# JuanDuGit/DH3D

Measured on AMD Instinct MI355X. Metric: point-clouds/sec, higher is better.
Workload: dtype f32; 1 GPU; local-descriptor forward (basic_config), N=8192 K=8, batch=8; clouds_per_gpu=8, clouds_total=8, points=8192, knn=8, parallelism=clouds sharded over 1 GPU(s), no data-path collective, weights=random-init (no checkpoint blobs exist upstream), steps_in_flight=4

## Files before the change

### dh3d_amd/_lib.py

```python
import ctypes
import os

import torch

_HERE = os.path.dirname(os.path.abspath(__file__))
LIB_PATH = os.environ.get("DH3D_HIP_LIB") or os.path.join(_HERE, "libdh3d_hip.so")

DH3D_OK = 0
ACT_NONE, ACT_RELU, ACT_SIGMOID = 0, 1, 2

_lib = None

c_fp = ctypes.c_void_p
c_int = ctypes.c_int
c_size_t = ctypes.c_size_t
c_float = ctypes.c_float
c_ll = ctypes.c_longlong
c_double = ctypes.c_double
c_u64 = ctypes.c_uint64


class Epilogue(ctypes.Structure):
    _fields_ = [("pre_bias", ctypes.c_void_p), ("scale", ctypes.c_void_p), ("shift", ctypes.c_void_p),
                ("act", ctypes.c_int)]
# ... 76 lines not shown
    "dh3d_netvlad_assign_rows_bwd": [c_fp, c_ll, c_int, c_fp, c_fp, c_fp, c_fp, c_fp, c_fp, c_fp],
    "dh3d_l2norm_rows_bwd": [c_fp, c_fp, c_ll, c_int, c_float, c_fp, c_fp],
    "dh3d_transpose32": [c_fp, c_int, c_int, c_int, c_fp, c_fp],
    "dh3d_colsum_f32": [c_fp, c_ll, c_int, c_int, c_fp, c_fp],
    "dh3d_farthest_point_sample": [c_int, c_int, c_int, c_fp, c_fp, c_fp, c_fp],
    "dh3d_farthest_point_sample_mode": [c_int, c_int, c_int, c_fp, c_fp, c_fp, c_int, c_fp],
    "dh3d_group_point_fwd": [c_int, c_int, c_int, c_int, c_int, c_fp, c_fp, c_fp, c_fp],
    "dh3d_group_point_bwd": [c_int, c_int, c_int, c_int, c_int, c_fp, c_fp, c_fp, c_fp],
    "dh3d_three_nn": [c_int, c_int, c_int, c_fp, c_fp, c_fp, c_fp, c_fp],
    "dh3d_three_interpolate_fwd": [c_int, c_int, c_int, c_int, c_fp, c_fp, c_fp, c_fp, c_fp],
    "dh3d_three_interpolate_bwd": [c_int, c_int, c_int, c_int, c_fp, c_fp, c_fp, c_fp, c_fp],
    "dh3d_spatial_sort": [c_fp, c_int, c_int, c_fp, c_fp, c_fp],
    "dh3d_knn_sorted": [c_fp, c_fp, c_int, c_int, c_int, c_fp, c_fp, c_fp],
    "dh3d_spatial_sort_cells": [c_fp, c_int, c_int, c_fp, c_fp, c_fp, c_fp],
    "dh3d_knn_grid": [c_fp, c_fp, c_fp, c_int, c_int, c_int, c_fp, c_fp, c_fp],
    "dh3d_knn_grid_plan": [c_int, c_int, c_int],
    "dh3d_fps_sorted": [c_fp, c_fp, c_int, c_int, c_int, c_fp, c_fp],
    "dh3d_three_nn_sorted": [c_int, c_int, c_int, c_fp, c_fp, c_fp, c_fp, c_fp, c_fp, c_fp],
    "dh3d_fps_sorted_xyz": [c_fp, c_fp, c_int, c_int, c_int, c_fp, c_fp, c_fp],
    "dh3d_fps_sorted_ordered": [c_fp, c_fp, c_fp, c_int, c_int, c_int, c_fp, c_fp, c_fp, c_fp, c_fp, c_fp],
    "dh3d_fps_sorted_cloud": [c_fp, c_fp, c_fp, c_int, c_int, c_int, c_fp, c_fp, c_fp],
    "dh3d_fps_sorted_fits": [c_int, c_int, c_int, c_int],
    "dh3d_pack_weight": [c_fp, c_int, c_int, c_fp, c_fp],
    "dh3d_pack_flex_weight": [c_fp, c_fp, c_int, c_int, c_fp, c_fp],
    "dh3d_flex_conv_pm_gather_fwd": [c_fp, c_fp, c_int, c_fp, c_fp, c_fp, c_int, c_int, c_int, c_int, c_int,
                                     ctypes.POINTER(Epilogue), c_fp, c_fp],
    "dh3d_flex_conv_pm_fwd": [c_fp, c_fp, c_fp, c_fp, c_int, c_int, c_int, c_int, c_int,
                              ctypes.POINTER(Epilogue), c_fp, c_fp],
    "dh3d_flex_conv_pm_tile_x6_fwd": [c_fp, c_fp, c_fp, c_fp, c_int, c_int, c_int, c_int, c_int, ctypes.POINTER(Epilogue), c_fp,
                                   c_fp, c_int, c_fp, c_fp],
# ... 42 lines not shown
    "dh3d_interp_bn_bwd_sums": [c_fp, c_int, c_int, c_fp, c_fp, c_fp, c_int, c_int, c_int, c_fp, c_fp, c_fp, c_fp, c_fp,
                                c_fp, c_fp, c_fp, c_fp],
    "dh3d_interp_bn_bwd_apply": [c_fp, c_int, c_int, c_fp, c_fp, c_fp, c_int, c_int, c_int, c_fp, c_fp, c_fp, c_fp, c_fp,
                                 c_fp, c_fp, c_fp, c_fp],
    "dh3d_linear_pm_x6_fwd": [c_fp, c_int, c_fp, c_int, c_fp, c_int, c_int, ctypes.POINTER(Epilogue), c_fp, c_fp, c_fp],
    "dh3d_se_res_pm_packed_fwd": [c_fp, c_fp, c_fp, c_fp, c_fp, c_fp, c_int, c_int, c_fp, c_fp],
    "dh3d_se_res_pool_pm_packed_fwd": [c_fp, c_fp, c_int, c_int, c_int, c_fp, c_fp, c_fp, c_fp, c_int, c_fp, c_fp],
    "dh3d_se_res_pool_conv_pm_fwd": [c_fp, c_fp, c_int, c_int, c_int, c_fp, c_fp, c_fp, c_fp, c_int, c_fp, c_fp,
                                     ctypes.POINTER(Epilogue), c_int, c_fp, c_fp],
    "dh3d_flex_pool_pm_fwd": [c_fp, c_fp, c_int, c_int, c_int, c_int, c_fp, c_fp, c_fp],
    "dh3d_flex_avg_pm_fwd": [c_fp, c_fp, c_int, c_int, c_int, c_int, c_float, c_fp, c_fp],
    "dh3d_conv_pointset_pm_fwd": [c_fp, c_fp, c_fp, c_fp, c_int, c_int, c_int, c_int, ctypes.POINTER(Epilogue),
                                  c_fp, c_fp],
    "dh3d_conv_pointset_pool_pm_fwd": [c_fp, c_fp, c_fp, c_fp, c_int, c_int, c_int, c_int, ctypes.POINTER(Epilogue),
                                       c_fp, c_fp, c_fp],
    "dh3d_linear_pm_fwd": [c_fp, c_int, c_fp, c_int, c_fp, c_int, c_int, ctypes.POINTER(Epilogue), c_fp, c_fp,
                           c_fp],
    "dh3d_se_res_pm_fwd": [c_fp, c_fp, c_fp, c_fp, c_fp, c_fp, c_int, c_int, c_fp, c_fp],
    "dh3d_three_interpolate_idw_fwd": [c_int, c_int, c_int, c_int, c_fp, c_fp, c_fp, c_fp, c_fp],
    "dh3d_l2norm_concat_fwd": [c_fp, c_int, c_int, c_float, c_fp, c_int, c_fp, c_fp],
    "dh3d_mlp_head_pm_fwd": [c_fp, c_int, c_int, c_fp, c_int, ctypes.POINTER(Epilogue), c_fp, c_float, c_fp,
                             c_fp],
    "dh3d_pack_weight_x3": [c_fp, c_int, c_int, c_fp, c_fp],
    "dh3d_mlp_head_pm_x6_fwd": [c_fp, c_int, c_int, c_fp, c_int, ctypes.POINTER(Epilogue), c_fp, c_float, c_fp,
                                c_fp],
    "dh3d_netvlad_workspace_bytes": [c_int, c_int, c_int, c_int],
    "dh3d_netvlad_aggregate_fwd": [c_fp, c_fp, c_fp, c_fp, c_fp, c_fp, c_int, c_int, c_int, c_int, c_fp,
                                   c_size_t, c_fp, c_fp],
    "dh3d_netvlad_head_workspace_bytes": [c_int, c_int, c_int],
    "dh3d_netvlad_tail_workspace_bytes": [c_int, c_int, c_int, c_int],
# ... 124 lines not shown
```

### dh3d_amd/backbones.py

```python
import math

import torch
from torch import nn

from . import _lib as L
from . import pm


class TPBatchNorm(nn.Module):

    ema_unbiased = True

    def __init__(self, channels, eps=1e-5):
        super().__init__()
        self.eps = eps
        self.gamma = nn.Parameter(torch.ones(channels))
        self.beta = nn.Parameter(torch.zeros(channels))
        self.register_buffer("mean_EMA", torch.zeros(channels))
        self.register_buffer("variance_EMA", torch.ones(channels))

    def fold(self):
        scale = self.gamma * torch.rsqrt(self.variance_EMA + self.eps)
        shift = self.beta - self.mean_EMA * scale
        return scale.contiguous(), shift.contiguous()
# ... 180 lines not shown
        cp = inner._prep or inner.prepare()
        if (packed is not None and x.dim() == 3 and x.shape[2] == 64 and inner.cin == 64 and inner.cout == 64
                and "wp" in cp and not cp.get("pad")):
            return pm.se_res_pool_conv(x, nbr, *packed, cp["wp"], cp["b"], cp["scale"], cp["shift"], act=act)
        y = self.forward_on_max_pool(x, nbr)
        return y, conv(y, act=act)


class Geometry(object):

    def __init__(self, xyz, knn_num, nbr=None, fps_contract=None):
        self.fps_contract = fps_contract
        self.xyz = xyz
        self.knn_num = knn_num
        self.nbr = nbr
        self.levels = {}
        self.sorted = None
        self.cells = None

    def ordered(self, cells=False):
        if self.sorted is None:
            if cells:
                srt, gbox, self.cells = pm.spatial_sort_cells(self.xyz)
                self.sorted = (srt, gbox)
            else:
                self.sorted = pm.spatial_sort(self.xyz)
        return self.sorted

    def level(self, dilate, knn, finish=True):
        key = (dilate, knn)
# ... 406 lines not shown
```

### dh3d_amd/csrc/flex_pm.hip

```cpp
#include <float.h>

#include "mfma_gemm.h"

namespace {

template <int DIN, int DOUT, int TMSEL = 0>
struct FlexCfg {
  static constexpr int TM = TMSEL ? TMSEL : (DIN <= 64 ? 64 : 32);
  static constexpr int KD = 4 * DIN;
  static constexpr int LD = KD + 4;
  static constexpr int MB = TM / 32;
  static constexpr int NB = DOUT / 32;
  static constexpr int NT = NB * MB / 4;
  static constexpr int LPR = DIN / 4;
  static constexpr int PPR = 256 / LPR;
  static constexpr int ROUNDS = TM / PPR;
  static_assert(NT >= 1 && NB * MB % 4 == 0, "tile must split over 4 waves");
};

template <int DIN, int DOUT, int KT, int TMSEL = 0>
__global__ __launch_bounds__(256) void flex_conv_pm_kernel(
    const float *__restrict__ feat, const float *__restrict__ xyz, const int32_t *__restrict__ nbr,
    const float *__restrict__ wpacked, long long R, int N, int K, EpilogueArgs ep,
    float *__restrict__ out, const int32_t *__restrict__ remap, int Nsrc) {
// ... 421 lines not shown
    hipLaunchKernelGGL(conv_pointset_pm_anyk_kernel, dim3(flat_grid(R * (Dout / 4))), dim3(256), 0,
                       (hipStream_t)stream, xyz, nbr, theta, bias, R, N, K, Dout, dh3d_ep(ep), out);
  }
  return dh3d_launch_status();
}

DH3D_API int dh3d_pointset_sum_pm(const float *xyz, const int32_t *nbr, int B, int N, int K, float *S, void *stream) {
  DH3D_REQUIRE(xyz && nbr && S && B > 0 && N > 0);
  DH3D_SUPPORTED(K == 8);
  const long long R = (long long)B * N;
  hipLaunchKernelGGL(pointset_sum_kernel, dim3(dh3d_cdiv(R, 256)), dim3(256), 0, (hipStream_t)stream, xyz, nbr, R, N,
                     reinterpret_cast<float4 *>(S));
  return dh3d_launch_status();
}

DH3D_API int dh3d_conv_pointset_pool_pm_fwd(const float *xyz, const int32_t *nbr, const float *theta, const float *bias,
                                            int B, int N, int K, int Dout, const dh3d_epilogue *ep, float *scratch,
                                            float *out, void *stream) {
  DH3D_REQUIRE(xyz && nbr && theta && bias && scratch && out && B > 0 && N > 0 && Dout > 0);
  DH3D_SUPPORTED(K == 8 && (Dout == 32 || Dout == 64 || Dout == 128) && (long long)B * N * (Dout / 4) < (1ll << 31));
  const long long R = (long long)B * N;
  hipStream_t s = (hipStream_t)stream;
  float4 *S = reinterpret_cast<float4 *>(scratch);
  hipLaunchKernelGGL(pointset_sum_kernel, dim3(dh3d_cdiv(R, 256)), dim3(256), 0, s, xyz, nbr, R, N, S);
  const dim3 grid(dh3d_cdiv(R * (Dout / 4), 256)), block(256);
  const EpilogueArgs e = dh3d_ep(ep);
  if (Dout == 32)
    hipLaunchKernelGGL(pointset_pool_kernel<8>, grid, block, 0, s, S, nbr, theta, bias, (int)R, N, e, out);
  else if (Dout == 64)
    hipLaunchKernelGGL(pointset_pool_kernel<16>, grid, block, 0, s, S, nbr, theta, bias, (int)R, N, e, out);
  else
    hipLaunchKernelGGL(pointset_pool_kernel<32>, grid, block, 0, s, S, nbr, theta, bias, (int)R, N, e, out);
  return dh3d_launch_status();
}
```

### dh3d_amd/csrc/knn.hip

```cpp
#include <float.h>
#include <limits.h>

#include <type_traits>

#include "common.h"
#include "wave_ops.h"

#pragma clang fp contract(off)

namespace {

typedef float f32x2 __attribute__((ext_vector_type(2)));
typedef unsigned long long u64;

constexpr int kQueriesPerBlock = 256;
constexpr int kChunk = 1024;
constexpr int kQueue = 16;

struct KnnLadder {
  int log2ct;
  int ctmask;
  int cv;
};

// ... 20 lines not shown
__device__ __forceinline__ int cand_slot(int c, int comp) {
  const int g = c >> 2, r = c & 3;
  const int off = (r < 2) ? (2 * comp + r) : (4 + 2 * comp + r);
  return g * 12 + off;
}

__device__ __forceinline__ float knn_bcast(float v, int lane) {
  return __int_as_float(__builtin_amdgcn_readlane(__float_as_int(v), lane));
}

__device__ __forceinline__ int knn_pick_near(unsigned long long m, int gl) {
  const unsigned long long up = m >> gl, dn = m & ((1ull << gl) - 1);
  const int da = up ? __builtin_ctzll(up) : 128;
  const int db = dn ? gl - (63 - __builtin_clzll(dn)) : 128;
  return da <= db ? gl + da : gl - db;
}

template <int KMAX>
struct KnnState {
  u64 keys[KMAX];
  float bound;
};

template <int KMAX, bool KEEP_MIN = false>
__device__ __forceinline__ void knn_insert_key(KnnState<KMAX> &st, const u64 key) {
  if (key < st.keys[KMAX - 1]) {
    if constexpr (KMAX <= 16) {
      bool lt[KMAX];
#pragma unroll
      for (int i = 0; i < KMAX - 1; ++i) lt[i] = key < st.keys[i];
// ... 317 lines not shown
          o_nn[i] = -1;
          o_d[i] = FLT_MAX;
        } else {
          o_nn[i] = (int)(((tb % (unsigned)lad.cv) << lad.log2ct) + tb / (unsigned)lad.cv);
          o_d[i] = __uint_as_float((unsigned)(st.keys[i] >> 32));
        }
      }
    }
  }
}

template <int S>
__host__ __device__ constexpr int knn_split_lds_bytes() {
  return S * (64 * 3 * 4 + kQueue * 64 * 8 + 64 * 4 + 64 * 4 + 64 * 4);
}
template <int KMAX, int S>
__device__ __forceinline__ void knn_split_body(const float4 *__restrict__ sorted, const float *__restrict__ gbox, int N, int K,
                                               const KnnLadder lad, int32_t *__restrict__ nn, float *__restrict__ dist,
                                               const int b, const int g, unsigned char *lds, const int wave0 = 0) {
  static_assert(KMAX * 64 * sizeof(u64) <= kQueue * 64 * sizeof(uint2), "a K-list fits its wave's survivor queue");
  uint2 (*s_q)[kQueue * 64] = reinterpret_cast<uint2 (*)[kQueue * 64]>(lds);
  float (*s_c)[64 * 3] = reinterpret_cast<float (*)[64 * 3]>(lds + S * kQueue * 64 * 8);
  int (*s_id)[64] = reinterpret_cast<int (*)[64]>(lds + S * (kQueue * 64 * 8 + 64 * 3 * 4));
  float (*s_share)[64] = reinterpret_cast<float (*)[64]>(lds + S * (kQueue * 64 * 8 + 64 * 3 * 4 + 64 * 4));
  float (*s_kth)[64] = reinterpret_cast<float (*)[64]>(lds + S * (kQueue * 64 * 8 + 64 * 3 * 4 + 64 * 8));
  constexpr int R = (KMAX + S - 1) / S - 1;
  const int lane = threadIdx.x & 63;
  const int wave = __builtin_amdgcn_readfirstlane((int)(threadIdx.x >> 6) - wave0);
  const int NG = (N + 63) / 64;
  const float4 *sc = sorted + (size_t)b * N;
  const float4 *gb = reinterpret_cast<const float4 *>(gbox) + (size_t)b * NG * 2;
  float *my_c = s_c[wave];
  uint2 *my_q = s_q[wave];
  int *my_id = s_id[wave];
// ... 197 lines not shown
          for (int t = KMAX - 1; t > 0; --t) {
            const u64 a = st.keys[t - 1], c = st.keys[t];
            const bool lt = c < a;
            st.keys[t - 1] = lt ? c : a;
            st.keys[t] = lt ? a : c;
          }
        }
      }
    }
  }

  if (wave == 0 && valid) {
    const int y = __float_as_int(qr.w);
    int32_t *o_nn = nn + ((size_t)b * N + y) * K;
    float *o_d = dist + ((size_t)b * N + y) * K;
#pragma unroll
    for (int i = 0; i < KMAX; ++i) {
      if (i < K) {
        const unsigned tb = (unsigned)st.keys[i];
        if (st.keys[i] == ~0ull) {
          o_nn[i] = -1;
          o_d[i] = FLT_MAX;
        } else {
          o_nn[i] = (int)(((tb % (unsigned)lad.cv) << lad.log2ct) + tb / (unsigned)lad.cv);
          o_d[i] = __uint_as_float((unsigned)(st.keys[i] >> 32));
        }
      }
    }
  }
}


template <int KMAX, int S>
__global__ __launch_bounds__(64 * S) void knn_split_kernel(const float4 *__restrict__ sorted,
                                                         const float *__restrict__ gbox, int N, int K,
                                                         KnnLadder lad, int32_t *__restrict__ nn,
                                                         float *__restrict__ dist, const int *__restrict__ gate) {
  if (gate && !gate[(size_t)blockIdx.y * kCellInts + kCellFlag]) return;
  __shared__ __attribute__((aligned(16))) unsigned char s_lds[knn_split_lds_bytes<S>()];
  const unsigned ng = (unsigned)((N + 63) / 64);
  knn_split_body<KMAX, S>(sorted, gbox, N, K, lad, nn, dist, blockIdx.y, (int)((blockIdx.x + 37u * blockIdx.y) % ng), s_lds);
}
// ... 205 lines not shown
__device__ __forceinline__ unsigned knn_spread4(unsigned v) {
  return (v & 1u) | ((v & 2u) << 2) | ((v & 4u) << 4) | ((v & 8u) << 6);
}
__device__ __forceinline__ void knn_cswap(u64 &a, u64 &b) {
  const bool lt = b < a;
  const u64 lo = lt ? b : a, hi = lt ? a : b;
  a = lo; b = hi;
}
template <int CTRL>
__device__ __forceinline__ u64 knn_dpp_u64(u64 v) {
  const int lo = __builtin_amdgcn_update_dpp(0, (int)(unsigned)v, CTRL, 0xF, 0xF, true);
  const int hi = __builtin_amdgcn_update_dpp(0, (int)(unsigned)(v >> 32), CTRL, 0xF, 0xF, true);
  return ((u64)(unsigned)hi << 32) | (unsigned)lo;
}
template <int CTRL>
__device__ __forceinline__ void knn_merge_step(KnnState<8> &st) {
  u64 c[8];
#pragma unroll
  for (int i = 0; i < 8; ++i) {
    const u64 mine = st.keys[i], theirs = knn_dpp_u64<CTRL>(st.keys[7 - i]);
    c[i] = mine < theirs ? mine : theirs;
  }
  knn_cswap(c[0], c[4]); knn_cswap(c[1], c[5]); knn_cswap(c[2], c[6]); knn_cswap(c[3], c[7]);
  knn_cswap(c[0], c[2]); knn_cswap(c[1], c[3]); knn_cswap(c[4], c[6]); knn_cswap(c[5], c[7]);
  knn_cswap(c[0], c[1]); knn_cswap(c[2], c[3]); knn_cswap(c[4], c[5]); knn_cswap(c[6], c[7]);
#pragma unroll
  for (int i = 0; i < 8; ++i) st.keys[i] = c[i];
}
template <int L>
__device__ __forceinline__ void knn_merge_sublanes(KnnState<8> &st) {
  if (L >= 2) knn_merge_step<0xB1>(st);
  if (L >= 4) knn_merge_step<0x4E>(st);
  if (L >= 8) knn_merge_step<0x141>(st);
  const unsigned hb = (unsigned)(st.keys[7] >> 32);
  if (hb <= 0x7f800000u) {
    const float dk = __uint_as_float(hb);
    st.bound = __fmul_rn(__fmul_rn(dk, dk), 1.000001f);
  }
}

template <int L, int SF>
__global__ __launch_bounds__(256) void knn_grid_kernel(const float4 *__restrict__ sorted, const float *__restrict__ gbox,
                                                      const int *__restrict__ cells, int N, int K, int D, KnnLadder lad,
                                                      int32_t *__restrict__ nn, float *__restrict__ dist) {
  constexpr int QB = 256 / L;
  static_assert(SF == 0 || (L == 4 && SF <= 4), "the merged scan: 64 queries per workgroup, at most four waves");
  constexpr int kGridLds = 3 * 64 * 4 + QB * kGridCap * 2 + QB * 4;
  constexpr int kSplitLds = SF == 2 ? 2 * knn_split_lds_bytes<2>() : SF > 0 ? knn_split_lds_bytes<(SF > 0 ? SF : 1)>() : 0;
  __shared__ __attribute__((aligned(16))) unsigned char s_raw[kGridLds > kSplitLds ? kGridLds : kSplitLds];
  const int b = blockIdx.y, lane = threadIdx.x & 63, sub = lane & (L - 1);
  if (cells[(size_t)b * kCellInts + kCellFlag]) {
    if constexpr (SF > 0) {
      const int ngq = (N + 63) / 64;
      if constexpr (SF == 2) {
        const int half = (int)(threadIdx.x >> 7), pairs = (ngq + 1) / 2;
        if ((int)blockIdx.x >= pairs) return;
        const int g0 = (int)blockIdx.x + half * pairs;
        if (g0 >= ngq) return;
        knn_split_body<8, 2>(sorted, gbox, N, K, lad, nn, dist, b, (int)(((unsigned)g0 + 37u * (unsigned)b) % (unsigned)ngq),
                             s_raw + half * knn_split_lds_bytes<2>(), half * 2);
      } else if (threadIdx.x < 64 * SF) {
        knn_split_body<8, (SF > 0 ? SF : 1)>(sorted, gbox, N, K, lad, nn, dist, b, (int)((blockIdx.x + 37u * (unsigned)b) % (unsigned)ngq), s_raw);
      }
    }
    return;
  }
  const int qi = (int)((blockIdx.x + 37u * (unsigned)b) % gridDim.x) * QB + threadIdx.x / L;
  const bool valid = qi < N;
  const float4 *sc = sorted + (size_t)b * N;
  const int *ct = cells + (size_t)b * kCellInts;
  const float *hd = reinterpret_cast<const float *>(ct) + 4100;
  const float lo[3] = {hd[0], hd[1], hd[2]}, scl[3] = {hd[3], hd[4], hd[5]};
  const float4 qr = sc[valid ? qi : N - 1];
  const float q[3] = {qr.x, qr.y, qr.z};
  const unsigned sched = (unsigned)ct[4107];
  int nb[3] = {0, 0, 0}, drop[3] = {0, 0, 0};
#pragma unroll
// ... 85 lines not shown
  };
  auto drain = [&]() {
    __builtin_amdgcn_fence(__ATOMIC_SEQ_CST, "wavefront");
    __builtin_amdgcn_wave_barrier();
    const int total = min(s_cnt[qs], kGridCap);
#pragma unroll 1
    for (int base = sub; base < total; base += 4 * L) {
      float4 r[4];
      bool ok[4];
#pragma unroll
      for (int u = 0; u < 4; ++u) {
        const int i = base + u * L;
        ok[u] = i < total;
        r[u] = sc[s_list[qs][min(i, total - 1)]];
      }
#pragma unroll
      for (int u = 0; u < 4; ++u) {
        const float dx = r[u].x - q[0], dy = r[u].y - q[1], dz = r[u].z - q[2];
        const float s2 = fmaf(dz, dz, fmaf(dy, dy, dx * dx));
        knn_offer<8, false>(st, ok[u] ? s2 : __builtin_nanf(""), __float_as_int(r[u].w), lad);
      }
    }
    __builtin_amdgcn_fence(__ATOMIC_SEQ_CST, "wavefront");
    __builtin_amdgcn_wave_barrier();
  };
  auto column = [&](auto tmask, int dy, int dz) __attribute__((always_inline)) {
    constexpr int TMASK = decltype(tmask)::value;
    const int ay = cq[1] + dy - 2, az = cq[2] + dz - 2;
    if ((unsigned)ay > (unsigned)gmax[1] || (unsigned)az > (unsigned)gmax[2]) return;
    const float d2yz = axis_d2(1, dy - 2) + axis_d2(2, dz - 2);
    const unsigned bityz = cell_code(0, ay, az);
    int beg[5], end[5];
#pragma unroll
    for (int t = 0; t < 5; ++t)
      if (TMASK >> t & 1) {
// ... 90 lines not shown
#pragma unroll
          for (int u = 0; u < 8; ++u) r8[u] = sc[min(j + u, j1 - 1)];
#pragma unroll
          for (int u = 0; u < 8; ++u) {
            const float dx = r8[u].x - q[0], dy = r8[u].y - q[1], dz = r8[u].z - q[2];
            const float s2 = fmaf(dz, dz, fmaf(dy, dy, dx * dx));
            knn_offer<8, false>(st, j + u < j1 ? s2 : __builtin_nanf(""), __float_as_int(r8[u].w), lad);
          }
        }
      }
    }
    knn_merge_sublanes<L>(st);
  }
  if (valid) {
    const int y = __float_as_int(qr.w);
#pragma unroll
    for (int e = 0; e < 8 / L; ++e) {
      const int slot = e * L + sub;
      if (slot >= K) break;
      u64 key = st.keys[0];
#pragma unroll
      for (int i = 1; i < 8; ++i) key = slot == i ? st.keys[i] : key;
      const size_t o = ((size_t)b * N + y) * K + slot;
      if (key == ~0ull) {
        nn[o] = -1;
        dist[o] = FLT_MAX;
      } else {
        const unsigned tb = (unsigned)key;
        nn[o] = (int)(((tb % (unsigned)lad.cv) << lad.log2ct) + tb / (unsigned)lad.cv);
        dist[o] = __uint_as_float((unsigned)(key >> 32));
      }
    }
  }
}

constexpr int kGridLanes = 4;

struct KnnGridPlan {
  int sf, drop;
};
static KnnGridPlan knn_grid_plan(int B, int N) {
  KnnGridPlan p{0, 0};
  while (p.drop < 6 && ((long long)N << p.drop) <= 3072) ++p.drop;
  const long long groups = (long long)((N + 63) / 64) * B;
  if (kGridLanes == 4 && groups <= 4096) p.sf = groups > 1280 ? 2 : 4;
  return p;
}

DH3D_API int dh3d_knn_grid_plan(int B, int N, int K) {
  if (B <= 0 || N <= 0 || K <= 0 || K > 8 || N > 16384 || B > 65535) return -1;
  const KnnGridPlan p = knn_grid_plan(B, N);
  return p.sf + 16 * p.drop;
}

DH3D_API int dh3d_knn_grid(const float *sorted, const float *gbox, const int32_t *cells, int B, int N, int K, int32_t *nn,
                           float *dist, void *stream) {
  DH3D_REQUIRE(sorted && gbox && cells && nn && dist && B > 0 && N > 0 && K > 0);
  DH3D_SUPPORTED(K <= 8 && N <= 16384 && B <= 65535);
  const KnnLadder lad = knn_ladder(N);
  constexpr int kLanes = kGridLanes;
  const KnnGridPlan plan = knn_grid_plan(B, N);
  const int D = plan.drop;
  const dim3 grid(dh3d_cdiv(N, 256 / kLanes), B);
  const float4 *so = reinterpret_cast<const float4 *>(sorted);
  if (plan.sf == 2) {
    hipLaunchKernelGGL((knn_grid_kernel<4, 2>), grid, dim3(256), 0, (hipStream_t)stream, so, gbox, cells, N, K, D, lad, nn, dist);
    return dh3d_launch_status();
  }
  if (plan.sf == 4) {
    hipLaunchKernelGGL((knn_grid_kernel<4, 4>), grid, dim3(256), 0, (hipStream_t)stream, so, gbox, cells, N, K, D, lad, nn, dist);
    return dh3d_launch_status();
  }
  hipLaunchKernelGGL((knn_grid_kernel<kLanes, 0>), grid, dim3(256), 0, (hipStream_t)stream, so, gbox, cells, N, K, D, lad, nn, dist);
  if (dh3d_launch_status() != DH3D_OK) return DH3D_ERR_LAUNCH;
  return knn_sorted_launch(sorted, gbox, B, N, K, nn, dist, cells, stream);
}
```

### dh3d_amd/model.py

```python

import torch
from torch import nn

from . import backbones as bb
from . import pm
from .configs import ConfigFactory, dotdict


def tf_variable_name(state_dict_key):
    name = state_dict_key.replace(".", "/")
    name = name.replace("mean_EMA", "mean/EMA").replace("variance_EMA", "variance/EMA")
    return name


def _copy_in(src, dst):
    if (not src.is_cuda and src.is_pinned() and src.is_contiguous() and src.dtype == dst.dtype
            and src.numel() == dst.numel()):
        pm.stage_copy(src, dst)
    else:
        dst.copy_(src, non_blocking=True)


def _capture_warmed(body, warmup, device):
    s = torch.cuda.Stream(device=device)
# ... 186 lines not shown
                geo._tail_accum = torch.zeros((pm.global_tail_accum_size(points.shape[0], points.shape[1] // 8),),
                                              dtype=torch.float32, device=points.device)
            if getattr(self, "steps_in_flight", 1) > 1:
                geo.busy_cus_per_xcd = min(8, (self.steps_in_flight - 1) * ((points.shape[0] + 7) // 8))
        else:
            geo.busy_cus_per_xcd = min(8, getattr(self, "steps_in_flight", 1) * ((points.shape[0] + 7) // 8))
        side.wait_event(fork)
        with torch.cuda.stream(side):
            if knn_inds is not None:
                geo.nbr = knn_inds.contiguous()
            elif points.shape[1] > 16384:
                geo.nbr, _ = pm.knn_xyz(points, self.knn_num)
            else:
                srt, gbox = geo.ordered()
                if geo.cells is not None:
                    geo.nbr, _ = pm.knn_grid(srt, gbox, geo.cells, self.knn_num)
                else:
                    geo.nbr, _ = pm.knn_sorted(srt, gbox, self.knn_num)
            geo.nbr.record_stream(main)
        return geo

    def _three_nn_before_sampled_level(self, points):
        return getattr(self, "steps_in_flight", 1) > 1

    def _join_side(self, geo):
        torch.cuda.current_stream().wait_stream(geo._side)

    def compute_local(self, points, knn_inds=None, _geo=None, _l2cat_eps=None, _prezero_tail=False):
        self._check_mode(need_head=False)
        geo = _geo if _geo is not None else self._geometry(points, knn_inds)
        main = torch.cuda.current_stream()
        p = self._local._prep
        with torch.cuda.stream(geo._side):
            nn_8 = geo.nbr if geo.nbr.shape[2] == 8 else geo.nbr[:, :, 0:8].contiguous()
            if nn_8.shape[2] == 8 and p["theta"].shape[1] in (32, 64, 128):
                init = pm.conv_pointset_pool_xyz(geo.xyz, nn_8, p["theta"], p["bias"], scale=p["scale"], shift=p["shift"],
                                                 act=pm.ACT_RELU)
            else:
                init = pm.flex_pool(pm.conv_pointset_xyz(geo.xyz, nn_8, p["theta"], p["bias"], scale=p["scale"],
                                                         shift=p["shift"], act=pm.ACT_RELU), nn_8)
            fuse_sc = points.shape[1] <= 4096 and self.stage2.shortcut_fusable(points.shape[1])
            r = self.stage1(geo, init, nbr=nn_8, post_conv=self.before_stage2_conv1d)
            x1, x2 = r if isinstance(r, tuple) else (r, self.before_stage2_conv1d(r, act=pm.ACT_RELU))
            cconv = self.stage2.concat_conv1d.tfconv0 if getattr(self.stage2, "concat", False) else None
            small = points.shape[1] <= 4096
            fused_tail = ((_l2cat_eps is not None or small) and cconv is not None
                          and self._local.featdim == 128 and cconv.commuted_supported(128)
                          and cconv.tail_fusable(self.local_stage1_shortcut.tfconv0, points.shape[1],
                                                 in_flight=getattr(self, "steps_in_flight", 1) > 1))
            if fused_tail:
                fuse_sc = False
            shortcut = lower = None
# ... 199 lines not shown
```

### dh3d_amd/pm.py

```python

import torch

from . import _lib as L

ACT_NONE, ACT_RELU, ACT_SIGMOID = L.ACT_NONE, L.ACT_RELU, L.ACT_SIGMOID


def knn_xyz(xyz, k):
    x = L.require_cuda_f32(xyz, "xyz", 3)
    B, N, _ = x.shape
    nn = torch.empty((B, N, k), dtype=torch.int32, device=x.device)
    dist = torch.empty((B, N, k), dtype=torch.float32, device=x.device)
    L.check(L.lib().dh3d_knn_bruteforce_xyz(L.ptr(x), B, N, k, L.ptr(nn), L.ptr(dist), L.stream_ptr()), "knn_xyz")
    return nn, dist


def spatial_sort(xyz):
    x = L.require_cuda_f32(xyz, "xyz", 3)
    B, N, _ = x.shape
    srt = torch.empty((B, N, 4), dtype=torch.float32, device=x.device)
    gbox = torch.empty((B, (N + 63) // 64, 8), dtype=torch.float32, device=x.device)
    L.check(L.lib().dh3d_spatial_sort(L.ptr(x), B, N, L.ptr(srt), L.ptr(gbox), L.stream_ptr()), "spatial_sort")
    return srt, gbox

# ... 13 lines not shown


def knn_grid(srt, gbox, cells, k, out=None):
    B, N, _ = srt.shape
    if out is None:
        nn = torch.empty((B, N, k), dtype=torch.int32, device=srt.device)
        dist = torch.empty((B, N, k), dtype=torch.float32, device=srt.device)
    else:
        nn, dist = out
        for t, dt, name in ((nn, torch.int32, "nn"), (dist, torch.float32, "dist")):
            if tuple(t.shape) != (B, N, k) or t.dtype != dt or t.device != srt.device or not t.is_contiguous():
                raise ValueError("knn_grid: out %s must be contiguous %s [%d, %d, %d] on %s, got %s %s on %s"
                                 % (name, dt, B, N, k, srt.device, t.dtype, tuple(t.shape), t.device))
    L.check(L.lib().dh3d_knn_grid(L.ptr(srt), L.ptr(gbox), L.ptr(cells), B, N, k, L.ptr(nn), L.ptr(dist), L.stream_ptr()), "knn_grid")
    return nn, dist


def knn_grid_plan(B, N, k):
    r = L.lib().dh3d_knn_grid_plan(int(B), int(N), int(k))
    return None if r < 0 else (r % 16, r // 16)


def knn_sorted(srt, gbox, k):
    B, N, _ = srt.shape
    nn = torch.empty((B, N, k), dtype=torch.int32, device=srt.device)
    dist = torch.empty((B, N, k), dtype=torch.float32, device=srt.device)
    L.check(L.lib().dh3d_knn_sorted(L.ptr(srt), L.ptr(gbox), B, N, k, L.ptr(nn), L.ptr(dist), L.stream_ptr()),
            "knn_sorted")
    return nn, dist

# ... 207 lines not shown


def conv_pointset_xyz(xyz, nbr, theta, bias, pre_bias=None, scale=None, shift=None, act=ACT_NONE):
    x = L.require_cuda_f32(xyz, "xyz", 3)
    nb = L.require_cuda_i32(nbr, "nbr", 3)
    B, N, _ = x.shape
    K = nb.shape[2]
    Dout = theta.shape[1]
    out = torch.empty((B, N, Dout), dtype=torch.float32, device=x.device)
    ep = L.make_epilogue(pre_bias, scale, shift, act)
    L.check(L.lib().dh3d_conv_pointset_pm_fwd(L.ptr(x), L.ptr(nb), L.ptr(theta), L.ptr(bias), B, N, K, Dout, ep,
                                              L.ptr(out), L.stream_ptr()), "conv_pointset_pm")
    return out


def conv_pointset_pool_xyz(xyz, nbr, theta, bias, pre_bias=None, scale=None, shift=None, act=ACT_NONE):
    x = L.require_cuda_f32(xyz, "xyz", 3)
    nb = L.require_cuda_i32(nbr, "nbr", 3)
    B, N, _ = x.shape
    Dout = theta.shape[1]
    out = torch.empty((B, N, Dout), dtype=torch.float32, device=x.device)
    scratch = torch.empty((B, N, 4), dtype=torch.float32, device=x.device)
    ep = L.make_epilogue(pre_bias, scale, shift, act)
    L.check(L.lib().dh3d_conv_pointset_pool_pm_fwd(L.ptr(x), L.ptr(nb), L.ptr(theta), L.ptr(bias), B, N, nb.shape[2], Dout,
                                                   ep, L.ptr(scratch), L.ptr(out), L.stream_ptr()), "conv_pointset_pool_pm")
    return out


def linear(x1, wpacked, Dout, x2=None, pre_bias=None, scale=None, shift=None, act=ACT_NONE, residual=None):
    a = L.require_cuda_f32(x1, "x1")
    lead = a.shape[:-1]
    C1 = a.shape[-1]
    R = a.numel() // C1
    C2 = 0
    b = None
    if x2 is not None:
        b = L.require_cuda_f32(x2, "x2")
        C2 = b.shape[-1]
# ... 804 lines not shown
```

### include/dh3d_hip.h

```cpp
#ifndef DH3D_HIP_H_
#define DH3D_HIP_H_

#include <stddef.h>
#include <stdint.h>

#ifdef __cplusplus
extern "C" {
#endif

#define DH3D_OK 0
#define DH3D_ERR_INVALID_ARGUMENT 1
#define DH3D_ERR_UNSUPPORTED 2
#define DH3D_ERR_LAUNCH 3

#define DH3D_ACT_NONE 0
#define DH3D_ACT_RELU 1
#define DH3D_ACT_SIGMOID 2

int dh3d_version(void);
#define DH3D_ABI_VERSION 4
int dh3d_abi_version(void);
const char *dh3d_arch(void);
const char *dh3d_source_hash(void);
const char *dh3d_status_string(int st);
// ... 115 lines not shown

int dh3d_pack_weight(const float *W, int Kd, int Dout, float *packed, void *stream);
int dh3d_pack_flex_weight(const float *theta, const float *bias, int Din, int Dout, float *packed,
                          void *stream);

int dh3d_spatial_sort(const float *xyz, int B, int N, float *sorted, float *gbox, void *stream);

int dh3d_knn_sorted(const float *sorted, const float *gbox, int B, int N, int K, int32_t *nn, float *dist,
                    void *stream);

#define DH3D_CELL_INTS 4112
int dh3d_spatial_sort_cells(const float *xyz, int B, int N, float *sorted, float *gbox, int32_t *cells, void *stream);

int dh3d_knn_grid(const float *sorted, const float *gbox, const int32_t *cells, int B, int N, int K, int32_t *nn, float *dist,
                  void *stream);
int dh3d_knn_grid_plan(int B, int N, int K);


int dh3d_three_nn_sorted(int b, int n, int m, const float *sorted1, const float *gbox1, const float *sorted2,
                         const float *gbox2, float *dist, int32_t *idx, void *stream);

int dh3d_fps_sorted(const float *sorted, const float *gbox, int B, int N, int m, int32_t *out, void *stream);
int dh3d_fps_sorted_xyz(const float *sorted, const float *gbox, int B, int N, int m, int32_t *out, float *xyz_out,
                        void *stream);
int dh3d_fps_sorted_ordered(const float *sorted, const float *gbox, const int32_t *cells, int B, int N, int m, int32_t *out,
                            float *xyz_out, float *sorted_s, float *gbox_s, int32_t *cells_s, void *stream);
int dh3d_fps_sorted_cloud(const float *sorted, const float *gbox, const float *xyz, int B, int N, int m, int32_t *out,
                          float *xyz_out, void *stream);
int dh3d_fps_sorted_fits(int N, int m, int ordered, int with_cloud);

// ... 20 lines not shown
int dh3d_flex_pool_pm_fwd(const float *features, const int32_t *nbr, int B, int N, int K, int C,
                          float *out, int32_t *argmax, void *stream);

int dh3d_flex_avg_pm_fwd(const float *features, const int32_t *nbr, int B, int N, int K, int C,
                         float scale, float *out, void *stream);

int dh3d_conv_pointset_pm_fwd(const float *xyz, const int32_t *nbr, const float *theta,
                              const float *bias, int B, int N, int K, int Dout,
                              const dh3d_epilogue *ep, float *out, void *stream);

int dh3d_pointset_sum_pm(const float *xyz, const int32_t *nbr, int B, int N, int K, float *S, void *stream);

int dh3d_conv_pointset_pool_pm_fwd(const float *xyz, const int32_t *nbr, const float *theta, const float *bias, int B,
                                   int N, int K, int Dout, const dh3d_epilogue *ep, float *scratch, float *out,
                                   void *stream);

int dh3d_linear_pm_fwd(const float *x1, int C1, const float *x2, int C2, const float *wpacked,
                       int R, int Dout, const dh3d_epilogue *ep, const float *residual, float *out,
                       void *stream);

int dh3d_se_res_pm_fwd(const float *x, const float *pool, const float *W1, const float *b1,
                       const float *W2, const float *b2, int R, int C, float *out, void *stream);
int dh3d_se_res_pm_packed_fwd(const float *x, const float *pool, const float *w1packed, const float *b1pad,
                              const float *w2packed, const float *b2, int R, int C, float *out, void *stream);
int dh3d_se_res_pool_pm_packed_fwd(const float *x, const int32_t *nbr, int B, int N, int K, const float *w1packed,
                                   const float *b1pad, const float *w2packed, const float *b2, int C, float *out,
                                   void *stream);
int dh3d_se_res_pool_conv_pm_fwd(const float *x, const int32_t *nbr, int B, int N, int K, const float *w1packed,
                                 const float *b1pad, const float *w2packed, const float *b2, int C, float *out,
                                 const float *wconv_packed, const dh3d_epilogue *ep, int Dout, float *out2, void *stream);
// ... 205 lines not shown
```

Baseline: 38160 point-clouds/sec.

## Fuse neighbour point-sum computation into grid kNN kernel epilogue

The grid kNN kernel gains a variant that, once each query's eight neighbours are found, gathers their coordinates (via DPP lane broadcast across the four sublanes) and writes the per-point offset sums. The pointset-conv pool then consumes those sums directly and skips its separate pointset_sum kernel launch and its re-gather of neighbour xyz. The crowded-cloud inner loop also changes from offering candidates one at a time to a bound-filtered four-candidate sorting-network merge that is skipped when no lane has a surviving candidate. This adds work and registers to the kNN kernel epilogue in exchange for removing one launch and one pass over memory.

```diff
diff --git a/dh3d_amd/_lib.py b/dh3d_amd/_lib.py
--- a/dh3d_amd/_lib.py
+++ b/dh3d_amd/_lib.py
@@ -114,6 +114,7 @@
     "dh3d_knn_sorted": [c_fp, c_fp, c_int, c_int, c_int, c_fp, c_fp, c_fp],
     "dh3d_spatial_sort_cells": [c_fp, c_int, c_int, c_fp, c_fp, c_fp, c_fp],
     "dh3d_knn_grid": [c_fp, c_fp, c_fp, c_int, c_int, c_int, c_fp, c_fp, c_fp],
+    "dh3d_knn_grid_sums": [c_fp, c_fp, c_fp, c_int, c_int, c_int, c_fp, c_fp, c_fp, c_fp, c_fp],
     "dh3d_knn_grid_plan": [c_int, c_int, c_int],
     "dh3d_fps_sorted": [c_fp, c_fp, c_int, c_int, c_int, c_fp, c_fp],
     "dh3d_three_nn_sorted": [c_int, c_int, c_int, c_fp, c_fp, c_fp, c_fp, c_fp, c_fp, c_fp],
@@ -186,6 +187,8 @@
                                   c_fp, c_fp],
     "dh3d_conv_pointset_pool_pm_fwd": [c_fp, c_fp, c_fp, c_fp, c_int, c_int, c_int, c_int, ctypes.POINTER(Epilogue),
                                        c_fp, c_fp, c_fp],
+    "dh3d_pointset_pool_pm_fwd": [c_fp, c_fp, c_fp, c_fp, c_int, c_int, c_int, c_int, ctypes.POINTER(Epilogue), c_fp,
+                                  c_fp],
     "dh3d_linear_pm_fwd": [c_fp, c_int, c_fp, c_int, c_fp, c_int, c_int, ctypes.POINTER(Epilogue), c_fp, c_fp,
                            c_fp],
     "dh3d_se_res_pm_fwd": [c_fp, c_fp, c_fp, c_fp, c_fp, c_fp, c_int, c_int, c_fp, c_fp],
diff --git a/dh3d_amd/backbones.py b/dh3d_amd/backbones.py
--- a/dh3d_amd/backbones.py
+++ b/dh3d_amd/backbones.py
@@ -218,6 +218,7 @@
         self.xyz = xyz
         self.knn_num = knn_num
         self.nbr = nbr
+        self.nbr_sums = None
         self.levels = {}
         self.sorted = None
         self.cells = None
diff --git a/dh3d_amd/csrc/flex_pm.hip b/dh3d_amd/csrc/flex_pm.hip
--- a/dh3d_amd/csrc/flex_pm.hip
+++ b/dh3d_amd/csrc/flex_pm.hip
@@ -459,15 +459,14 @@
   return dh3d_launch_status();
 }
 
-DH3D_API int dh3d_conv_pointset_pool_pm_fwd(const float *xyz, const int32_t *nbr, const float *theta, const float *bias,
-                                            int B, int N, int K, int Dout, const dh3d_epilogue *ep, float *scratch,
-                                            float *out, void *stream) {
-  DH3D_REQUIRE(xyz && nbr && theta && bias && scratch && out && B > 0 && N > 0 && Dout > 0);
+static int pointset_pool_launch(const float *xyz, float *sums, const int32_t *nbr, const float *theta, const float *bias, int B,
+                                int N, int K, int Dout, const dh3d_epilogue *ep, float *out, void *stream) {
+  DH3D_REQUIRE(sums && nbr && theta && bias && out && B > 0 && N > 0 && Dout > 0);
   DH3D_SUPPORTED(K == 8 && (Dout == 32 || Dout == 64 || Dout == 128) && (long long)B * N * (Dout / 4) < (1ll << 31));
   const long long R = (long long)B * N;
   hipStream_t s = (hipStream_t)stream;
-  float4 *S = reinterpret_cast<float4 *>(scratch);
-  hipLaunchKernelGGL(pointset_sum_kernel, dim3(dh3d_cdiv(R, 256)), dim3(256), 0, s, xyz, nbr, R, N, S);
+  float4 *S = reinterpret_cast<float4 *>(sums);
+  if (xyz) hipLaunchKernelGGL(pointset_sum_kernel, dim3(dh3d_cdiv(R, 256)), dim3(256), 0, s, xyz, nbr, R, N, S);
   const dim3 grid(dh3d_cdiv(R * (Dout / 4), 256)), block(256);
   const EpilogueArgs e = dh3d_ep(ep);
   if (Dout == 32)
@@ -478,3 +477,15 @@
     hipLaunchKernelGGL(pointset_pool_kernel<32>, grid, block, 0, s, S, nbr, theta, bias, (int)R, N, e, out);
   return dh3d_launch_status();
 }
+
+DH3D_API int dh3d_conv_pointset_pool_pm_fwd(const float *xyz, const int32_t *nbr, const float *theta, const float *bias,
+                                            int B, int N, int K, int Dout, const dh3d_epilogue *ep, float *scratch,
+                                            float *out, void *stream) {
+  DH3D_REQUIRE(xyz);
+  return pointset_pool_launch(xyz, scratch, nbr, theta, bias, B, N, K, Dout, ep, out, stream);
+}
+
+DH3D_API int dh3d_pointset_pool_pm_fwd(const float *S, const int32_t *nbr, const float *theta, const float *bias, int B,
+                                       int N, int K, int Dout, const dh3d_epilogue *ep, float *out, void *stream) {
+  return pointset_pool_launch(nullptr, const_cast<float *>(S), nbr, theta, bias, B, N, K, Dout, ep, out, stream);
+}
diff --git a/dh3d_amd/csrc/knn.hip b/dh3d_amd/csrc/knn.hip
--- a/dh3d_amd/csrc/knn.hip
+++ b/dh3d_amd/csrc/knn.hip
@@ -58,6 +58,13 @@
   const int da = up ? __builtin_ctzll(up) : 128;
   const int db = dn ? gl - (63 - __builtin_clzll(dn)) : 128;
   return da <= db ? gl + da : gl - db;
+}
+
+__device__ __forceinline__ float4 knn_point_sum(const float (&px)[8], const float (&py)[8], const float (&pz)[8]) {
+  float sx = 0.f, sy = 0.f, sz = 0.f;
+#pragma unroll
+  for (int k = 0; k < 8; ++k) { sx += px[k] - px[0]; sy += py[k] - py[0]; sz += pz[k] - pz[0]; }
+  return make_float4(sx, sy, sz, 0.f);
 }
 
 template <int KMAX>
@@ -405,10 +412,11 @@
 __host__ __device__ constexpr int knn_split_lds_bytes() {
   return S * (64 * 3 * 4 + kQueue * 64 * 8 + 64 * 4 + 64 * 4 + 64 * 4);
 }
-template <int KMAX, int S>
+template <int KMAX, int S, bool SUMS = false>
 __device__ __forceinline__ void knn_split_body(const float4 *__restrict__ sorted, const float *__restrict__ gbox, int N, int K,
                                                const KnnLadder lad, int32_t *__restrict__ nn, float *__restrict__ dist,
-                                               const int b, const int g, unsigned char *lds, const int wave0 = 0) {
+                                               const int b, const int g, unsigned char *lds, const int wave0 = 0,
+                                               const float *__restrict__ xyz = nullptr, float4 *__restrict__ sums = nullptr) {
   static_assert(KMAX * 64 * sizeof(u64) <= kQueue * 64 * sizeof(uint2), "a K-list fits its wave's survivor queue");
   uint2 (*s_q)[kQueue * 64] = reinterpret_cast<uint2 (*)[kQueue * 64]>(lds);
   float (*s_c)[64 * 3] = reinterpret_cast<float (*)[64 * 3]>(lds + S * kQueue * 64 * 8);
@@ -636,18 +644,31 @@
     const int y = __float_as_int(qr.w);
     int32_t *o_nn = nn + ((size_t)b * N + y) * K;
     float *o_d = dist + ((size_t)b * N + y) * K;
+    int ids[KMAX];
 #pragma unroll
     for (int i = 0; i < KMAX; ++i) {
+      ids[i] = -1;
       if (i < K) {
         const unsigned tb = (unsigned)st.keys[i];
         if (st.keys[i] == ~0ull) {
           o_nn[i] = -1;
           o_d[i] = FLT_MAX;
         } else {
-          o_nn[i] = (int)(((tb % (unsigned)lad.cv) << lad.log2ct) + tb / (unsigned)lad.cv);
+          o_nn[i] = ids[i] = (int)(((tb % (unsigned)lad.cv) << lad.log2ct) + tb / (unsigned)lad.cv);
           o_d[i] = __uint_as_float((unsigned)(st.keys[i] >> 32));
         }
       }
+    }
+    if constexpr (SUMS) {
+      static_assert(KMAX == 8, "the point sums are over eight neighbours");
+      const float *pc = xyz + (size_t)b * N * 3;
+      float px[8], py[8], pz[8];
+#pragma unroll
+      for (int k = 0; k < 8; ++k) {
+        const float *p = pc + (size_t)max(ids[k], 0) * 3;
+        px[k] = p[0]; py[k] = p[1]; pz[k] = p[2];
+      }
+      sums[(size_t)b * N + y] = knn_point_sum(px, py, pz);
     }
   }
 }
@@ -883,6 +904,10 @@
   return ((u64)(unsigned)hi << 32) | (unsigned)lo;
 }
 template <int CTRL>
+__device__ __forceinline__ float knn_dpp_f32(float v) {
+  return __int_as_float(__builtin_amdgcn_update_dpp(0, __float_as_int(v), CTRL, 0xF, 0xF, true));
+}
+template <int CTRL>
 __device__ __forceinline__ void knn_merge_step(KnnState<8> &st) {
   u64 c[8];
 #pragma unroll
@@ -895,6 +920,24 @@
   knn_cswap(c[0], c[1]); knn_cswap(c[2], c[3]); knn_cswap(c[4], c[5]); knn_cswap(c[6], c[7]);
 #pragma unroll
   for (int i = 0; i < 8; ++i) st.keys[i] = c[i];
+}
+__device__ __forceinline__ void knn_merge_four(KnnState<8> &st, u64 (&n)[4]) {
+  knn_cswap(n[0], n[1]); knn_cswap(n[2], n[3]); knn_cswap(n[0], n[2]); knn_cswap(n[1], n[3]); knn_cswap(n[1], n[2]);
+  u64 c[8];
+#pragma unroll
+  for (int i = 0; i < 4; ++i) c[i] = st.keys[i];
+#pragma unroll
+  for (int i = 4; i < 8; ++i) c[i] = st.keys[i] < n[7 - i] ? st.keys[i] : n[7 - i];
+  knn_cswap(c[0], c[4]); knn_cswap(c[1], c[5]); knn_cswap(c[2], c[6]); knn_cswap(c[3], c[7]);
+  knn_cswap(c[0], c[2]); knn_cswap(c[1], c[3]); knn_cswap(c[4], c[6]); knn_cswap(c[5], c[7]);
+  knn_cswap(c[0], c[1]); knn_cswap(c[2], c[3]); knn_cswap(c[4], c[5]); knn_cswap(c[6], c[7]);
+#pragma unroll
+  for (int i = 0; i < 8; ++i) st.keys[i] = c[i];
+  const unsigned hb = (unsigned)(st.keys[7] >> 32);
+  if (hb <= 0x7f800000u) {
+    const float dk = __uint_as_float(hb);
+    st.bound = __fmul_rn(__fmul_rn(dk, dk), 1.000001f);
+  }
 }
 template <int L>
 __device__ __forceinline__ void knn_merge_sublanes(KnnState<8> &st) {
@@ -908,10 +951,12 @@
   }
 }
 
-template <int L, int SF>
+template <int L, int SF, bool SUMS>
 __global__ __launch_bounds__(256) void knn_grid_kernel(const float4 *__restrict__ sorted, const float *__restrict__ gbox,
                                                       const int *__restrict__ cells, int N, int K, int D, KnnLadder lad,
-                                                      int32_t *__restrict__ nn, float *__restrict__ dist) {
+                                                      int32_t *__restrict__ nn, float *__restrict__ dist,
+                                                      const float *__restrict__ xyz, float4 *__restrict__ sums) {
+  static_assert(!SUMS || (L == 4 && SF > 0), "the point sums: four lanes per query, crowded clouds in the same launch");
   constexpr int QB = 256 / L;
   static_assert(SF == 0 || (L == 4 && SF <= 4), "the merged scan: 64 queries per workgroup, at most four waves");
   constexpr int kGridLds = 3 * 64 * 4 + QB * kGridCap * 2 + QB * 4;
@@ -926,10 +971,11 @@
         if ((int)blockIdx.x >= pairs) return;
         const int g0 = (int)blockIdx.x + half * pairs;
         if (g0 >= ngq) return;
-        knn_split_body<8, 2>(sorted, gbox, N, K, lad, nn, dist, b, (int)(((unsigned)g0 + 37u * (unsigned)b) % (unsigned)ngq),
-                             s_raw + half * knn_split_lds_bytes<2>(), half * 2);
+        knn_split_body<8, 2, SUMS>(sorted, gbox, N, K, lad, nn, dist, b, (int)(((unsigned)g0 + 37u * (unsigned)b) % (unsigned)ngq),
+                                   s_raw + half * knn_split_lds_bytes<2>(), half * 2, xyz, sums);
       } else if (threadIdx.x < 64 * SF) {
-        knn_split_body<8, (SF > 0 ? SF : 1)>(sorted, gbox, N, K, lad, nn, dist, b, (int)((blockIdx.x + 37u * (unsigned)b) % (unsigned)ngq), s_raw);
+        knn_split_body<8, (SF > 0 ? SF : 1), SUMS>(sorted, gbox, N, K, lad, nn, dist, b,
+                                                   (int)((blockIdx.x + 37u * (unsigned)b) % (unsigned)ngq), s_raw, 0, xyz, sums);
       }
     }
     return;
@@ -1045,11 +1091,24 @@
         ok[u] = i < total;
         r[u] = sc[s_list[qs][min(i, total - 1)]];
       }
+      float s2[4];
+      bool any = false;
 #pragma unroll
       for (int u = 0; u < 4; ++u) {
         const float dx = r[u].x - q[0], dy = r[u].y - q[1], dz = r[u].z - q[2];
-        const float s2 = fmaf(dz, dz, fmaf(dy, dy, dx * dx));
-        knn_offer<8, false>(st, ok[u] ? s2 : __builtin_nanf(""), __float_as_int(r[u].w), lad);
+        s2[u] = fmaf(dz, dz, fmaf(dy, dy, dx * dx));
+        ok[u] = ok[u] && s2[u] <= st.bound;
+        any = any || ok[u];
+      }
+      if (__any(any)) {
+        u64 nk[4];
+#pragma unroll
+        for (int u = 0; u < 4; ++u) {
+          const int x = __float_as_int(r[u].w);
+          const unsigned tb = (unsigned)((x & lad.ctmask) * lad.cv + (x >> lad.log2ct));
+          nk[u] = ok[u] ? ((u64)__float_as_uint(sqrtf(s2[u])) << 32) | tb : ~0ull;
+        }
+        knn_merge_four(st, nk);
       }
     }
     __builtin_amdgcn_fence(__ATOMIC_SEQ_CST, "wavefront");
@@ -1170,6 +1229,9 @@
   }
   if (valid) {
     const int y = __float_as_int(qr.w);
+    int ids[8 / L];
+#pragma unroll
+    for (int e = 0; e < 8 / L; ++e) ids[e] = -1;
 #pragma unroll
     for (int e = 0; e < 8 / L; ++e) {
       const int slot = e * L + sub;
@@ -1183,9 +1245,24 @@
         dist[o] = FLT_MAX;
       } else {
         const unsigned tb = (unsigned)key;
-        nn[o] = (int)(((tb % (unsigned)lad.cv) << lad.log2ct) + tb / (unsigned)lad.cv);
+        nn[o] = ids[e] = (int)(((tb % (unsigned)lad.cv) << lad.log2ct) + tb / (unsigned)lad.cv);
         dist[o] = __uint_as_float((unsigned)(key >> 32));
       }
+    }
+    if constexpr (SUMS) {
+      const float *pc = xyz + (size_t)b * N * 3;
+      const float *p0 = pc + (size_t)max(ids[0], 0) * 3, *p1 = pc + (size_t)max(ids[1], 0) * 3;
+      const float mx[2] = {p0[0], p1[0]}, my[2] = {p0[1], p1[1]}, mz[2] = {p0[2], p1[2]};
+      float px[8], py[8], pz[8];
+#pragma unroll
+      for (int e = 0; e < 2; ++e) {
+        px[4 * e + 0] = knn_dpp_f32<0x00>(mx[e]); py[4 * e + 0] = knn_dpp_f32<0x00>(my[e]); pz[4 * e + 0] = knn_dpp_f32<0x00>(mz[e]);
+        px[4 * e + 1] = knn_dpp_f32<0x55>(mx[e]); py[4 * e + 1] = knn_dpp_f32<0x55>(my[e]); pz[4 * e + 1] = knn_dpp_f32<0x55>(mz[e]);
+        px[4 * e + 2] = knn_dpp_f32<0xAA>(mx[e]); py[4 * e + 2] = knn_dpp_f32<0xAA>(my[e]); pz[4 * e + 2] = knn_dpp_f32<0xAA>(mz[e]);
+        px[4 * e + 3] = knn_dpp_f32<0xFF>(mx[e]); py[4 * e + 3] = knn_dpp_f32<0xFF>(my[e]); pz[4 * e + 3] = knn_dpp_f32<0xFF>(mz[e]);
+      }
+      const float4 sv = knn_point_sum(px, py, pz);
+      if (sub == 0) sums[(size_t)b * N + y] = sv;
     }
   }
 }
@@ -1209,25 +1286,46 @@
   return p.sf + 16 * p.drop;
 }
 
-DH3D_API int dh3d_knn_grid(const float *sorted, const float *gbox, const int32_t *cells, int B, int N, int K, int32_t *nn,
-                           float *dist, void *stream) {
-  DH3D_REQUIRE(sorted && gbox && cells && nn && dist && B > 0 && N > 0 && K > 0);
-  DH3D_SUPPORTED(K <= 8 && N <= 16384 && B <= 65535);
+static int knn_grid_launch(const float *sorted, const float *gbox, const int32_t *cells, int B, int N, int K, int32_t *nn,
+                           float *dist, const float *xyz, float *sums, void *stream) {
   const KnnLadder lad = knn_ladder(N);
   constexpr int kLanes = kGridLanes;
   const KnnGridPlan plan = knn_grid_plan(B, N);
   const int D = plan.drop;
   const dim3 grid(dh3d_cdiv(N, 256 / kLanes), B);
   const float4 *so = reinterpret_cast<const float4 *>(sorted);
+  float4 *S = reinterpret_cast<float4 *>(sums);
+  hipStream_t s = (hipStream_t)stream;
+  if (sums) {
+    if (plan.sf == 2) hipLaunchKernelGGL((knn_grid_kernel<4, 2, true>), grid, dim3(256), 0, s, so, gbox, cells, N, K, D, lad, nn, dist, xyz, S);
+    else hipLaunchKernelGGL((knn_grid_kernel<4, 4, true>), grid, dim3(256), 0, s, so, gbox, cells, N, K, D, lad, nn, dist, xyz, S);
+    return dh3d_launch_status();
+  }
+  const float *no_xyz = nullptr;
+  float4 *no_S = nullptr;
   if (plan.sf == 2) {
-    hipLaunchKernelGGL((knn_grid_kernel<4, 2>), grid, dim3(256), 0, (hipStream_t)stream, so, gbox, cells, N, K, D, lad, nn, dist);
+    hipLaunchKernelGGL((knn_grid_kernel<4, 2, false>), grid, dim3(256), 0, s, so, gbox, cells, N, K, D, lad, nn, dist, no_xyz, no_S);
     return dh3d_launch_status();
   }
   if (plan.sf == 4) {
-    hipLaunchKernelGGL((knn_grid_kernel<4, 4>), grid, dim3(256), 0, (hipStream_t)stream, so, gbox, cells, N, K, D, lad, nn, dist);
+    hipLaunchKernelGGL((knn_grid_kernel<4, 4, false>), grid, dim3(256), 0, s, so, gbox, cells, N, K, D, lad, nn, dist, no_xyz, no_S);
     return dh3d_launch_status();
   }
-  hipLaunchKernelGGL((knn_grid_kernel<kLanes, 0>), grid, dim3(256), 0, (hipStream_t)stream, so, gbox, cells, N, K, D, lad, nn, dist);
+  hipLaunchKernelGGL((knn_grid_kernel<kLanes, 0, false>), grid, dim3(256), 0, s, so, gbox, cells, N, K, D, lad, nn, dist, no_xyz, no_S);
   if (dh3d_launch_status() != DH3D_OK) return DH3D_ERR_LAUNCH;
   return knn_sorted_launch(sorted, gbox, B, N, K, nn, dist, cells, stream);
 }
+
+DH3D_API int dh3d_knn_grid(const float *sorted, const float *gbox, const int32_t *cells, int B, int N, int K, int32_t *nn,
+                           float *dist, void *stream) {
+  DH3D_REQUIRE(sorted && gbox && cells && nn && dist && B > 0 && N > 0 && K > 0);
+  DH3D_SUPPORTED(K <= 8 && N <= 16384 && B <= 65535);
+  return knn_grid_launch(sorted, gbox, cells, B, N, K, nn, dist, nullptr, nullptr, stream);
+}
+
+DH3D_API int dh3d_knn_grid_sums(const float *sorted, const float *gbox, const int32_t *cells, int B, int N, int K, int32_t *nn,
+                                float *dist, const float *xyz, float *S, void *stream) {
+  DH3D_REQUIRE(sorted && gbox && cells && nn && dist && xyz && S && B > 0 && N > 0 && K > 0);
+  DH3D_SUPPORTED(K == 8 && N >= 8 && N <= 16384 && B <= 65535 && knn_grid_plan(B, N).sf != 0);
+  return knn_grid_launch(sorted, gbox, cells, B, N, K, nn, dist, xyz, S, stream);
+}
diff --git a/dh3d_amd/model.py b/dh3d_amd/model.py
--- a/dh3d_amd/model.py
+++ b/dh3d_amd/model.py
@@ -224,7 +224,11 @@
             else:
                 srt, gbox = geo.ordered()
                 if geo.cells is not None:
-                    geo.nbr, _ = pm.knn_grid(srt, gbox, geo.cells, self.knn_num)
+                    B, N = points.shape[0], points.shape[1]
+                    if self.knn_num == 8 and N >= 8 and pm.knn_grid_plan(B, N, 8)[0] != 0:
+                        geo.nbr, _, geo.nbr_sums = pm.knn_grid_sums(srt, gbox, geo.cells, points, 8)
+                    else:
+                        geo.nbr, _ = pm.knn_grid(srt, gbox, geo.cells, self.knn_num)
                 else:
                     geo.nbr, _ = pm.knn_sorted(srt, gbox, self.knn_num)
             geo.nbr.record_stream(main)
@@ -245,7 +249,7 @@
             nn_8 = geo.nbr if geo.nbr.shape[2] == 8 else geo.nbr[:, :, 0:8].contiguous()
             if nn_8.shape[2] == 8 and p["theta"].shape[1] in (32, 64, 128):
                 init = pm.conv_pointset_pool_xyz(geo.xyz, nn_8, p["theta"], p["bias"], scale=p["scale"], shift=p["shift"],
-                                                 act=pm.ACT_RELU)
+                                                 act=pm.ACT_RELU, sums=geo.nbr_sums if nn_8 is geo.nbr else None)
             else:
                 init = pm.flex_pool(pm.conv_pointset_xyz(geo.xyz, nn_8, p["theta"], p["bias"], scale=p["scale"],
                                                          shift=p["shift"], act=pm.ACT_RELU), nn_8)
diff --git a/dh3d_amd/pm.py b/dh3d_amd/pm.py
--- a/dh3d_amd/pm.py
+++ b/dh3d_amd/pm.py
@@ -51,6 +51,19 @@
                                  % (name, dt, B, N, k, srt.device, t.dtype, tuple(t.shape), t.device))
     L.check(L.lib().dh3d_knn_grid(L.ptr(srt), L.ptr(gbox), L.ptr(cells), B, N, k, L.ptr(nn), L.ptr(dist), L.stream_ptr()), "knn_grid")
     return nn, dist
+
+
+def knn_grid_sums(srt, gbox, cells, xyz, k=8):
+    x = L.require_cuda_f32(xyz, "xyz", 3)
+    B, N, _ = srt.shape
+    if tuple(x.shape) != (B, N, 3):
+        raise ValueError("knn_grid_sums: xyz %s is not the sorted cloud's [%d, %d, 3]" % (tuple(x.shape), B, N))
+    nn = torch.empty((B, N, k), dtype=torch.int32, device=srt.device)
+    dist = torch.empty((B, N, k), dtype=torch.float32, device=srt.device)
+    S = torch.empty((B, N, 4), dtype=torch.float32, device=srt.device)
+    L.check(L.lib().dh3d_knn_grid_sums(L.ptr(srt), L.ptr(gbox), L.ptr(cells), B, N, k, L.ptr(nn), L.ptr(dist), L.ptr(x), L.ptr(S),
+                                       L.stream_ptr()), "knn_grid_sums")
+    return nn, dist, S
 
 
 def knn_grid_plan(B, N, k):
@@ -288,14 +301,21 @@
     return out
 
 
-def conv_pointset_pool_xyz(xyz, nbr, theta, bias, pre_bias=None, scale=None, shift=None, act=ACT_NONE):
+def conv_pointset_pool_xyz(xyz, nbr, theta, bias, pre_bias=None, scale=None, shift=None, act=ACT_NONE, sums=None):
     x = L.require_cuda_f32(xyz, "xyz", 3)
     nb = L.require_cuda_i32(nbr, "nbr", 3)
     B, N, _ = x.shape
     Dout = theta.shape[1]
     out = torch.empty((B, N, Dout), dtype=torch.float32, device=x.device)
+    ep = L.make_epilogue(pre_bias, scale, shift, act)
+    if sums is not None:
+        S = L.require_cuda_f32(sums, "sums", 3)
+        if tuple(S.shape) != (B, N, 4):
+            raise ValueError("conv_pointset_pool_xyz: sums %s is not [%d, %d, 4]" % (tuple(S.shape), B, N))
+        L.check(L.lib().dh3d_pointset_pool_pm_fwd(L.ptr(S), L.ptr(nb), L.ptr(theta), L.ptr(bias), B, N, nb.shape[2], Dout, ep,
+                                                  L.ptr(out), L.stream_ptr()), "pointset_pool_pm")
+        return out
     scratch = torch.empty((B, N, 4), dtype=torch.float32, device=x.device)
-    ep = L.make_epilogue(pre_bias, scale, shift, act)
     L.check(L.lib().dh3d_conv_pointset_pool_pm_fwd(L.ptr(x), L.ptr(nb), L.ptr(theta), L.ptr(bias), B, N, nb.shape[2], Dout,
                                                    ep, L.ptr(scratch), L.ptr(out), L.stream_ptr()), "conv_pointset_pool_pm")
     return out
diff --git a/include/dh3d_hip.h b/include/dh3d_hip.h
--- a/include/dh3d_hip.h
+++ b/include/dh3d_hip.h
@@ -153,6 +153,8 @@
 
 int dh3d_knn_grid(const float *sorted, const float *gbox, const int32_t *cells, int B, int N, int K, int32_t *nn, float *dist,
                   void *stream);
+int dh3d_knn_grid_sums(const float *sorted, const float *gbox, const int32_t *cells, int B, int N, int K, int32_t *nn,
+                       float *dist, const float *xyz, float *S, void *stream);
 int dh3d_knn_grid_plan(int B, int N, int K);
 
 
@@ -203,6 +205,8 @@
 int dh3d_conv_pointset_pool_pm_fwd(const float *xyz, const int32_t *nbr, const float *theta, const float *bias, int B,
                                    int N, int K, int Dout, const dh3d_epilogue *ep, float *scratch, float *out,
                                    void *stream);
+int dh3d_pointset_pool_pm_fwd(const float *S, const int32_t *nbr, const float *theta, const float *bias, int B, int N,
+                              int K, int Dout, const dh3d_epilogue *ep, float *out, void *stream);
 
 int dh3d_linear_pm_fwd(const float *x1, int C1, const float *x2, int C2, const float *wpacked,
                        int R, int Dout, const dh3d_epilogue *ep, const float *residual, float *out,
```

New measurement: 38490 point-clouds/sec (median of 6 runs). Within noise of the previous version (+0.9%).
